# HyHuang1995/sp_orb_slam

Measured on AMD Instinct MI355X. Metric: frames/sec SuperPoint extract (752x480, 1k kpts), higher is better.
Workload: dtype f32

## Files before the change

### sp_orb_slam_amd/csrc/conv_f32.hip

```cpp
#include <type_traits>
#include <utility>

#include "spfe_kernels.h"
#include "../../include/spfe_exact_math.h"

namespace spfe {

typedef float f32x16 __attribute__((ext_vector_type(16)));

template <int KS, int TH>
struct Geo {
  static constexpr int HALO = KS / 2;
  static constexpr int ROWS = TH + 2 * HALO;
  static constexpr int COLS = 32 + 2 * HALO;
  static constexpr int ROWP = (KS == 3) ? 36 : 32;
  static constexpr int PLANE_RAW = ROWS * ROWP;
  static constexpr int PLANE = PLANE_RAW + ((2 - PLANE_RAW % 8) + 8) % 8;
};

typedef int i32x4 __attribute__((ext_vector_type(4)));
#define SPFE_OOB 0x80000000u

template <int NITER, int NWITER>
struct Pipe {
  float4 va[NITER];
  float4 vw[NWITER];
  int dst[NITER];
  unsigned voff[NITER];
  unsigned woff[NWITER];
  __amdgpu_buffer_rsrc_t rin, rw;
  const float *at[8];
  const float *bBase;
  float *nA, *nW;
};

template <int NR, int NT>
struct EpiCtx {
  __amdgpu_buffer_rsrc_t rout;
  unsigned rbase[NR][NT];
  float bias[NT];
  int xlim;
  unsigned pixstep;
};

__device__ __forceinline__ float max4_finite(float a, float b, float c, float d) {
  float m;
  asm("v_max3_f32 %0, %1, %2, %3\n\tv_max_f32 %0, %0, %4" : "=&v"(m) : "v"(a), "v"(b), "v"(c), "v"(d));
  return m;
}

template <int MT, int NT, bool POOL, bool RELU, int E>
__device__ __forceinline__ void epi_store(const EpiCtx<POOL ? MT / 2 : MT, NT> &e, const f32x16 (&acc)[MT][NT]) {
  constexpr int NEPI_ = POOL ? (MT / 2) * NT * 8 : MT * NT * 16;
  if constexpr (E >= NEPI_) {
    return;
  } else if constexpr (!POOL) {
    constexpr int j = E / (MT * 16), i = (E / 16) % MT, r = E % 16;
    constexpr int xr = (r & 3) + 8 * (r >> 2);
    float v = acc[i][j][r] + e.bias[j];
    if (RELU) v = v > 0.0f ? v : 0.0f;
    const unsigned off = xr < e.xlim ? e.rbase[i][j] : SPFE_OOB;
    __builtin_amdgcn_raw_buffer_store_b32(__float_as_int(v), e.rout, off, xr * e.pixstep, 0);
  } else {
    constexpr int ip = E / (NT * 8), j = (E / 8) % NT, r = 2 * (E % 8), i0 = 2 * ip;
    constexpr int xr = (r & 3) + 8 * (r >> 2);
    const float m = max4_finite(acc[i0][j][r], acc[i0][j][r + 1], acc[i0 + 1][j][r], acc[i0 + 1][j][r + 1]);
    float v = m + e.bias[j];
    if (RELU) v = v > 0.0f ? v : 0.0f;
    const unsigned off = xr < e.xlim ? e.rbase[ip][j] : SPFE_OOB;
    __builtin_amdgcn_raw_buffer_store_b32(__float_as_int(v), e.rout, off, (xr >> 1) * e.pixstep, 0);
  }
}

constexpr int F1_PROWS = 12, F1_PCOLS = 36, F1_PATCH = F1_PROWS * F1_PCOLS;

template <int NITER>
struct Fuse1a {
  float4 w[9], bias;
  float px[9];
  float4 o;
  unsigned pb[NITER];
  const float *patch;
  float *patch_next;
  const float *wsrc;
  const float *bsrc;
  __amdgpu_buffer_rsrc_t rimg;
  unsigned poff[2];
  unsigned pidx[2];
  unsigned pval[2];
  bool fill;
};
struct NoFuse {};

constexpr int F1_SUBS = 10;
template <int NITER, int IT, int SUB, int PLANE, int NWITER>
__device__ __forceinline__ void fuse_piece(Fuse1a<NITER> &z, Pipe<NITER, NWITER> &c) {
  if constexpr (SUB == 0) {
    const unsigned b = z.pb[IT] == ~0u ? 0u : z.pb[IT];
#pragma unroll
    for (int t = 0; t < 9; ++t) z.px[t] = z.patch[b + (t / 3) * F1_PCOLS + t % 3];
  } else if constexpr (SUB <= 8) {
    constexpr int j = (SUB - 1) / 2, half = (SUB - 1) % 2;
    float acc = half == 0 ? 0.0f : (j == 0 ? z.o.x : (j == 1 ? z.o.y : (j == 2 ? z.o.z : z.o.w)));
#pragma unroll
    for (int t = half * 5; t < (half == 0 ? 5 : 9); ++t) {
      const float wt = j == 0 ? z.w[t].x : (j == 1 ? z.w[t].y : (j == 2 ? z.w[t].z : z.w[t].w));
      acc = __builtin_fmaf(z.px[t], wt, acc);
    }
    if constexpr (half == 1) {
      const float bj = j == 0 ? z.bias.x : (j == 1 ? z.bias.y : (j == 2 ? z.bias.z : z.bias.w));
      acc = acc + bj;
      acc = acc > 0.0f ? acc : 0.0f;
      if (c.voff[IT] == SPFE_OOB) acc = 0.0f;
    }
    if constexpr (j == 0) z.o.x = acc;
    else if constexpr (j == 1) z.o.y = acc;
    else if constexpr (j == 2) z.o.z = acc;
    else z.o.w = acc;
  } else {
    float *d = c.nA + c.dst[IT];
    d[0] = z.o.x;
    d[PLANE] = z.o.y;
    d[2 * PLANE] = z.o.z;
    d[3 * PLANE] = z.o.w;
  }
}

template <int STEP, int NSTEP, bool FIRST, int KC, int KS, int MT, int NT, int PLANE, int ROWP, int NITER,
          int NWITER, bool POOL, bool RELU, bool FUSE, class FZ>
__device__ __forceinline__ void k_steps(float (&a)[2][MT], float (&bb)[2][NT], f32x16 (&acc)[MT][NT],
                                        const f32x16 (&accPrev)[MT][NT], Pipe<NITER, NWITER> &c,
                                        const EpiCtx<POOL ? MT / 2 : MT, NT> &e, FZ &fz) {
  if constexpr (STEP < NSTEP) {
    constexpr int NLDA = FUSE ? 0 : NITER;
    constexpr int NLD = NLDA + NWITER;
    constexpr int L0 = 1, W0 = NSTEP - NLD - 1;
    constexpr int NEPI = POOL ? (MT / 2) * NT * 8 : MT * NT * 16;
    constexpr int EPS = (NEPI + (NSTEP - 3)) / (NSTEP - 2);
    constexpr int cur = STEP & 1, nxt = cur ^ 1;
    static_assert(L0 + NLD <= W0, "loads and LDS writes of a stage must not overlap");
    constexpr int M = MT * NT;
    if constexpr (STEP >= 1) __builtin_amdgcn_s_waitcnt(0xC07F);
#pragma unroll
    for (int m = 0; m < M; ++m) {
      if (m == 0) {
        if constexpr (STEP + 1 < NSTEP) {
          constexpr int tap = (STEP + 1) / (KC / 2), t = (STEP + 1) % (KC / 2);
          constexpr int dy = tap / KS, dx = tap % KS;
#pragma unroll
          for (int i = 0; i < MT; ++i) {
            if constexpr (KC / 2 <= 8) a[nxt][i] = c.at[t][(i + dy) * ROWP + dx];
            else a[nxt][i] = c.at[0][(2 * t) * PLANE + (i + dy) * ROWP + dx];
          }
#pragma unroll
          for (int j = 0; j < NT; ++j) bb[nxt][j] = c.bBase[j * (KS * KS * KC * 32) + (tap * KC + 2 * t) * 32];
        }
      }
      if (m == 1 % M) {
        if constexpr (STEP >= L0 && STEP - L0 < NLD) {
          constexpr int it = STEP - L0;
          if constexpr (it < NLDA) {
            const i32x4 v = __builtin_amdgcn_raw_buffer_load_b128(c.rin, c.voff[it], 0, 0);
            c.va[it] = make_float4(__int_as_float(v.x), __int_as_float(v.y), __int_as_float(v.z), __int_as_float(v.w));
          } else {
            constexpr int wi = it - NLDA;
            const i32x4 v = __builtin_amdgcn_raw_buffer_load_b128(c.rw, c.woff[wi], 0, 0);
            c.vw[wi] = make_float4(__int_as_float(v.x), __int_as_float(v.y), __int_as_float(v.z), __int_as_float(v.w));
          }
        }
      }
      if (m == 2 % M) {
        if constexpr (FIRST && STEP >= 1) {
          constexpr int e0 = (STEP - 1) * EPS;
          [&]<int... Qs>(std::integer_sequence<int, Qs...>) {
            (epi_store<MT, NT, POOL, RELU, e0 + Qs>(e, accPrev), ...);
          }(std::make_integer_sequence<int, EPS>{});
        }
      }
      if (m == 3 % M) {
        if constexpr (STEP >= W0 && STEP - W0 < NLD) {
          constexpr int it = STEP - W0;
          if constexpr (it < NLDA) {
            float *d = c.nA + c.dst[it];
            d[0] = c.va[it].x;
            d[PLANE] = c.va[it].y;
            d[2 * PLANE] = c.va[it].z;
            d[3 * PLANE] = c.va[it].w;
          } else {
            constexpr int wi = it - NLDA;
            *reinterpret_cast<float4 *>(reinterpret_cast<char *>(c.nW) + c.woff[wi]) = c.vw[wi];
          }
        }
      }
      if (m == 1 % M) {
        if constexpr (FUSE) {
          constexpr int F0 = 12;
          static_assert(L0 + NLD <= F0 && F0 + F1_SUBS * NITER <= NSTEP, "fused conv1a schedule does not fit the stage");
          if constexpr (STEP >= F0 && STEP < F0 + F1_SUBS * NITER)
            fuse_piece<NITER, (STEP - F0) / F1_SUBS, (STEP - F0) % F1_SUBS, PLANE, NWITER>(fz, c);
        }
      }
      if (m == 3 % M) {
        if constexpr (FUSE) {
          static_assert(58 < W0, "fused conv1a schedule does not fit the stage");
          if constexpr (STEP >= 2 && STEP < 11) fz.w[STEP - 2] = *reinterpret_cast<const float4 *>(fz.wsrc + (STEP - 2) * 64);
          if constexpr (STEP == 11) fz.bias = *reinterpret_cast<const float4 *>(fz.bsrc);
          if constexpr (STEP == 50) {
            if (fz.fill) {
              fz.pval[0] = __builtin_amdgcn_raw_buffer_load_b8(fz.rimg, fz.poff[0], 0, 0);
              fz.pval[1] = __builtin_amdgcn_raw_buffer_load_b8(fz.rimg, fz.poff[1], 0, 0);
            }
          }
          if constexpr (STEP == 58) {
            if (fz.fill) {
              if (fz.pidx[0] < F1_PATCH) fz.patch_next[fz.pidx[0]] = spfe_pixel_to_float((uint8_t)fz.pval[0]);
              if (fz.pidx[1] < F1_PATCH) fz.patch_next[fz.pidx[1]] = spfe_pixel_to_float((uint8_t)fz.pval[1]);
            }
          }
        }
      }
      __builtin_amdgcn_sched_barrier(0);
      {
        const int i = m / NT, j = m % NT;
        if constexpr (FIRST && STEP == 0) {
          f32x16 z;
#pragma unroll
          for (int r = 0; r < 16; ++r) z[r] = 0.0f;
          acc[i][j] = __builtin_amdgcn_mfma_f32_32x32x2f32(a[cur][i], bb[cur][j], z, 0, 0, 0);
        } else {
          acc[i][j] = __builtin_amdgcn_mfma_f32_32x32x2f32(a[cur][i], bb[cur][j], acc[i][j], 0, 0, 0);
        }
      }
      __builtin_amdgcn_sched_barrier(0);
    }
    k_steps<STEP + 1, NSTEP, FIRST, KC, KS, MT, NT, PLANE, ROWP, NITER, NWITER, POOL, RELU, FUSE, FZ>(a, bb, acc, accPrev, c, e, fz);
  }
}

template <int LAYER, int CIN, int KS, int KC, int WM, int WN, int MT, int NT, bool POOL, bool RELU>
__global__ __launch_bounds__(64 * WM * WN, 1) void conv_f32_kernel(ConvParams p) {
  constexpr int TH = WM * MT;
  using G = Geo<KS, TH>;
  constexpr int TAPS = KS * KS;
  constexpr int NCHUNK = CIN / KC;
  constexpr int PLANE = G::PLANE;
  constexpr int ROWP = G::ROWP;
  constexpr int BUF = KC * PLANE + TAPS * KC * 64;
  static_assert(WM * WN == 4 || WM * WN == 8, "4 or 8 waves per workgroup");
  constexpr int NTHR = 64 * WM * WN;
  static_assert(WN * NT == 2, "64 output channels per workgroup");
  static_assert(!POOL || MT % 2 == 0, "pooling needs row pairs per wave");
  static_assert((KC * PLANE) % 4 == 0 && BUF % 4 == 0, "weight slabs must stay 16B aligned");
  constexpr int Q = KC / 4;
  constexpr int NITEM = G::ROWS * G::COLS * Q;
  constexpr int NITER = (NITEM + NTHR - 1) / NTHR;
  constexpr int NW4 = TAPS * KC * 16;
  constexpr int NWITER = (NW4 + NTHR - 1) / NTHR;
  constexpr int NSTEP = TAPS * (KC / 2);
  constexpr int SLAB_BYTES = TAPS * KC * 64 * 4;

  constexpr bool FUSE = LAYER == 2;
  static_assert(!FUSE || (CIN == 64 && KS == 3 && KC == 16 && TH == 8), "fused conv1a is conv1b's first operand");
  using FZ = typename std::conditional<FUSE, Fuse1a<NITER>, NoFuse>::type;

  extern __shared__ __attribute__((aligned(16))) float smem[];

  const int tid = threadIdx.x;
  const int lane = tid & 63;
  const int wave = __builtin_amdgcn_readfirstlane(tid >> 6);
  const int hi = lane >> 5, l31 = lane & 31;
  const int wm = wave % WM, wn = wave / WM;
  const int H = p.H, W = p.W;

  const int total = p.nblk * p.tiles_x * p.tiles_y * p.B;
  const int first = p.item_lo, count = (p.item_hi > 0 ? p.item_hi : total) - first;
  const int xcd = blockIdx.x & 7, gi = blockIdx.x >> 3, gper = gridDim.x >> 3;
  const int lo = first + (int)((long)count * xcd / 8), hi_w = first + (int)((long)count * (xcd + 1) / 8);
  int w = lo + gi;
  if (w >= hi_w) return;

  int i_nb, i_tx, i_ty, i_b;
  {
    int t = w;
    i_nb = t % p.nblk; t /= p.nblk;
    i_tx = t % p.tiles_x; t /= p.tiles_x;
    i_ty = t % p.tiles_y; i_b = t / p.tiles_y;
  }
  int d_nb, d_tx, d_ty, d_b;
  {
    int t = gper;
    d_nb = t % p.nblk; t /= p.nblk;
    d_tx = t % p.tiles_x; t /= p.tiles_x;
    d_ty = t % p.tiles_y; d_b = t / p.tiles_y;
  }

  const unsigned in_pix_bytes = (unsigned)p.in_stride * 4u;
  const unsigned frame_in_bytes = (unsigned)H * W * in_pix_bytes;
  const int Ho = POOL ? H >> 1 : H, Wo = POOL ? W >> 1 : W;
  const unsigned out_pix_bytes = (unsigned)p.out_stride * 4u;
  const unsigned frame_out_bytes = (unsigned)Ho * Wo * out_pix_bytes;

  Pipe<NITER, NWITER> c;
  int prow[NITER], pcol[NITER];
  unsigned pqb[NITER];
#pragma unroll
  for (int it = 0; it < NITER; ++it) {
    const int i = tid + it * NTHR;
    const int qq = i % Q, pix = i / Q;
    prow[it] = i < NITEM ? pix / G::COLS - G::HALO : (1 << 20);
    pcol[it] = pix % G::COLS - G::HALO;
    pqb[it] = qq * 16;
    c.dst[it] = i < NITEM ? (qq * 4) * PLANE + (pix / G::COLS) * ROWP + pix % G::COLS
                          : (ROWP > G::COLS ? (tid % G::ROWS) * ROWP + G::COLS : G::PLANE_RAW);
  }
#pragma unroll
  for (int it = 0; it < NWITER; ++it) c.woff[it] = ((tid + it * NTHR) % NW4) * 16;

  auto aim_tile = [&](int tx, int ty) {
#pragma unroll
    for (int it = 0; it < NITER; ++it) {
      const int gy = ty * TH + prow[it], gx = tx * 32 + pcol[it];
      c.voff[it] = ((unsigned)gy < (unsigned)H && (unsigned)gx < (unsigned)W)
                       ? (unsigned)(gy * W + gx) * in_pix_bytes + pqb[it]
                       : SPFE_OOB;
    }
  };
  auto aim_stage = [&](int nb, int b, int chunk, bool valid) {
    const float *base = p.in + (size_t)b * H * W * p.in_stride + p.in_choff + chunk * KC;
    c.rin = __builtin_amdgcn_make_buffer_rsrc(const_cast<float *>(base), 0, valid ? frame_in_bytes : 0u, 0x00020000);
    const float *wb = p.wpack + ((size_t)nb * NCHUNK + chunk) * (TAPS * KC * 64);
    c.rw = __builtin_amdgcn_make_buffer_rsrc(const_cast<float *>(wb), 0, valid ? (unsigned)SLAB_BYTES : 0u, 0x00020000);
  };

  aim_tile(i_tx, i_ty);
  aim_stage(i_nb, i_b, 0, true);
  FZ fz;
  [[maybe_unused]] float *sP = smem + 2 * BUF;
  [[maybe_unused]] int pcur = 0;
  [[maybe_unused]] int php[2] = {0, 0}, pwp[2] = {0, 0};
  if constexpr (FUSE) {
    const int qq = tid % Q;
#pragma unroll
    for (int it = 0; it < NITER; ++it) {
      const int i = tid + it * 256, pix = i / Q;
      fz.pb[it] = i < NITEM ? (unsigned)((pix / G::COLS) * F1_PCOLS + pix % G::COLS) : ~0u;
    }
#pragma unroll
    for (int k = 0; k < 2; ++k) {
      const int i = tid + k * 256;
      fz.pidx[k] = i < F1_PATCH ? (unsigned)i : 0xffffu;
      php[k] = i / F1_PCOLS;
      pwp[k] = i % F1_PCOLS;
      fz.poff[k] = SPFE_OOB;
      fz.pval[k] = 0u;
    }
    fz.fill = false;
    fz.patch = sP;
    fz.patch_next = sP + F1_PATCH;
    fz.rimg = __builtin_amdgcn_make_buffer_rsrc(const_cast<uint8_t *>(p.img), 0, 0u, 0x00020000);
    fz.wsrc = p.w1a + qq * 4;
    fz.bsrc = p.b1a + qq * 4;
    {
      const uint8_t *ib = p.img + (size_t)i_b * H * W;
#pragma unroll
      for (int k = 0; k < 2; ++k) {
        const int gy = i_ty * TH - 2 + php[k], gx = i_tx * 32 - 2 + pwp[k];
        const bool in = (unsigned)gy < (unsigned)H && (unsigned)gx < (unsigned)W;
        if (fz.pidx[k] < F1_PATCH) sP[fz.pidx[k]] = in ? spfe_pixel_to_float(ib[(size_t)gy * W + gx]) : 0.0f;
      }
    }
    __syncthreads();
#pragma unroll
    for (int t = 0; t < 9; ++t) fz.w[t] = *reinterpret_cast<const float4 *>(fz.wsrc + t * 64);
    fz.bias = *reinterpret_cast<const float4 *>(fz.bsrc);
    c.nA = smem;
    [&]<int... I>(std::integer_sequence<int, I...>) {
      (fuse_piece<NITER, I / F1_SUBS, I % F1_SUBS, PLANE, NWITER>(fz, c), ...);
    }(std::make_integer_sequence<int, F1_SUBS * NITER>{});
  } else {
#pragma unroll
    for (int it = 0; it < NITER; ++it) {
      const i32x4 v = __builtin_amdgcn_raw_buffer_load_b128(c.rin, c.voff[it], 0, 0);
      c.va[it] = make_float4(__int_as_float(v.x), __int_as_float(v.y), __int_as_float(v.z), __int_as_float(v.w));
    }
  }
#pragma unroll
  for (int it = 0; it < NWITER; ++it) {
    const i32x4 v = __builtin_amdgcn_raw_buffer_load_b128(c.rw, c.woff[it], 0, 0);
    c.vw[it] = make_float4(__int_as_float(v.x), __int_as_float(v.y), __int_as_float(v.z), __int_as_float(v.w));
  }
  if constexpr (!FUSE) {
#pragma unroll
    for (int it = 0; it < NITER; ++it) {
      float *d = smem + c.dst[it];
      d[0] = c.va[it].x;
      d[PLANE] = c.va[it].y;
      d[2 * PLANE] = c.va[it].z;
      d[3 * PLANE] = c.va[it].w;
    }
  }
#pragma unroll
  for (int it = 0; it < NWITER; ++it)
    *reinterpret_cast<float4 *>(reinterpret_cast<char *>(smem + KC * PLANE) + c.woff[it]) = c.vw[it];
  __syncthreads();

  f32x16 accA[MT][NT], accB[MT][NT];
#pragma unroll
  for (int i = 0; i < MT; ++i)
#pragma unroll
    for (int j = 0; j < NT; ++j)
#pragma unroll
      for (int r = 0; r < 16; ++r) { accA[i][j][r] = 0.0f; accB[i][j][r] = 0.0f; }

  constexpr int NR = POOL ? MT / 2 : MT;
  using Epi = EpiCtx<NR, NT>;
  Epi epi;
  epi.rout = __builtin_amdgcn_make_buffer_rsrc(p.out, 0, 0u, 0x00020000);
#pragma unroll
  for (int j = 0; j < NT; ++j) {
    epi.bias[j] = 0.0f;
#pragma unroll
    for (int q = 0; q < NR; ++q) epi.rbase[q][j] = SPFE_OOB;
  }
  epi.xlim = 0; epi.pixstep = out_pix_bytes;
  bool more = true;

  auto aim_epi = [&](Epi &e, int nb, int tx, int ty, int b) {
    float *obase = p.out + (size_t)b * Ho * Wo * p.out_stride + p.out_choff;
    e.rout = __builtin_amdgcn_make_buffer_rsrc(obase, 0, frame_out_bytes, 0x00020000);
    const int y0 = ty * TH + wm * MT, x0 = tx * 32 + 4 * hi;
    e.xlim = W - x0;
    e.pixstep = out_pix_bytes;
    const int ylim = H - y0;
    const unsigned rowstep = (unsigned)Wo * out_pix_bytes;
#pragma unroll
    for (int j = 0; j < NT; ++j) {
      const int co = nb * 64 + (wn * NT + j) * 32 + l31;
      const unsigned pix = POOL ? (unsigned)((y0 >> 1) * Wo + (x0 >> 1)) : (unsigned)(y0 * W + x0);
      const unsigned obase = pix * out_pix_bytes + (unsigned)co * 4u;
#pragma unroll
      for (int q = 0; q < NR; ++q)
        e.rbase[q][j] = (co < p.cout_real && (POOL ? 2 * q : q) < ylim) ? obase + q * rowstep : SPFE_OOB;
      e.bias[j] = p.bias[co];
    }
  };

  Epi epi_next;
  auto run_tile = [&](f32x16(&acc)[MT][NT], const f32x16(&accPrev)[MT][NT]) {
    int n_nb = i_nb + d_nb, n_tx = i_tx + d_tx, n_ty = i_ty + d_ty, n_b = i_b + d_b;
    if (n_nb >= p.nblk) { n_nb -= p.nblk; ++n_tx; }
    if (n_tx >= p.tiles_x) { n_tx -= p.tiles_x; ++n_ty; }
    if (n_ty >= p.tiles_y) { n_ty -= p.tiles_y; ++n_b; }
    const bool have_next_item = w + gper < hi_w;
    aim_epi(epi_next, i_nb, i_tx, i_ty, i_b);
    auto stage = [&]<bool FIRST>(std::bool_constant<FIRST>, const int chunk) {
      const bool last = chunk == NCHUNK - 1;
      if (!last) {
        aim_stage(i_nb, i_b, chunk + 1, true);
      } else {
        aim_tile(n_tx, n_ty);
        aim_stage(n_nb, n_b, 0, have_next_item);
      }
      if constexpr (FUSE) {
        const int produced = last ? 0 : chunk + 1;
        const int qq = tid % Q;
        fz.wsrc = p.w1a + produced * KC + qq * 4;
        fz.bsrc = p.b1a + produced * KC + qq * 4;
        fz.patch = sP + (last ? pcur ^ 1 : pcur) * F1_PATCH;
        fz.patch_next = sP + (pcur ^ 1) * F1_PATCH;
        fz.fill = chunk == NCHUNK - 2 && have_next_item;
        if (fz.fill) {
          fz.rimg = __builtin_amdgcn_make_buffer_rsrc(const_cast<uint8_t *>(p.img) + (size_t)n_b * H * W, 0,
                                                      (unsigned)(H * W), 0x00020000);
#pragma unroll
          for (int k = 0; k < 2; ++k) {
            const int gy = n_ty * TH - 2 + php[k], gx = n_tx * 32 - 2 + pwp[k];
            fz.poff[k] = ((unsigned)gy < (unsigned)H && (unsigned)gx < (unsigned)W) ? (unsigned)(gy * W + gx) : SPFE_OOB;
          }
        }
      }
      const int buf = chunk & 1;
      float *cA = smem + buf * BUF;
      c.nA = smem + (buf ^ 1) * BUF;
      c.nW = c.nA + KC * PLANE;
#pragma unroll
      for (int t = 0; t < (KC / 2 <= 8 ? KC / 2 : 1); ++t)
        c.at[t] = cA + (2 * t + hi) * PLANE + (wm * MT) * ROWP + l31;
      c.bBase = cA + KC * PLANE + (wn * NT) * (TAPS * KC * 32) + hi * 32 + l31;
      float a[2][MT], bb[2][NT];
#pragma unroll
      for (int i = 0; i < MT; ++i) a[0][i] = c.at[0][i * ROWP];
#pragma unroll
      for (int j = 0; j < NT; ++j) bb[0][j] = c.bBase[j * (TAPS * KC * 32)];
      k_steps<0, NSTEP, FIRST, KC, KS, MT, NT, PLANE, ROWP, NITER, NWITER, POOL, RELU, FUSE, FZ>(a, bb, acc, accPrev, c, epi, fz);
      __syncthreads();
    };
    static_assert(NCHUNK >= 2 && NCHUNK % 2 == 0, "the stage that carries the epilogue is not the tile's last; buf = chunk & 1");
    stage(std::true_type{}, 0);
#pragma unroll 1
    for (int chunk = 1; chunk < NCHUNK; ++chunk) stage(std::false_type{}, chunk);
    epi = epi_next;
    if constexpr (FUSE) pcur ^= 1;
    more = have_next_item;
    w += gper;
    i_nb = n_nb; i_tx = n_tx; i_ty = n_ty; i_b = n_b;
  };

  bool lastA = true;
  while (true) {
    run_tile(accA, accB);
    lastA = true;
    if (!more) break;
    run_tile(accB, accA);
    lastA = false;
    if (!more) break;
  }
  {
    constexpr int NEPI = POOL ? (MT / 2) * NT * 8 : MT * NT * 16;
    auto flush = [&](const f32x16(&acc)[MT][NT]) {
      [&]<int... E>(std::integer_sequence<int, E...>) {
        (epi_store<MT, NT, POOL, RELU, E>(epi, acc), ...);
      }(std::make_integer_sequence<int, NEPI>{});
    };
    if (lastA) flush(accA); else flush(accB);
  }
}

template <int LAYER, int CIN, int KS, int KC, int WM, int WN, int MT, int NT, bool POOL, bool RELU>
static hipError_t launch_one(const ConvParams &p, hipStream_t s) {
  constexpr int TH = WM * MT;
  using G = Geo<KS, TH>;
  constexpr size_t lds = (2 * (size_t)(KC * G::PLANE + KS * KS * KC * 64) + (LAYER == 2 ? 2 * F1_PATCH : 0)) * sizeof(float);
  static_assert(lds <= 160 * 1024, "double buffer must fit the 160 KB LDS");
  auto k = conv_f32_kernel<LAYER, CIN, KS, KC, WM, WN, MT, NT, POOL, RELU>;
  static bool attr_done[64] = {};
  int dev = 0;
  (void)hipGetDevice(&dev);
  if (dev < 0 || dev >= 64 || !attr_done[dev]) {
    hipError_t e = hipFuncSetAttribute(reinterpret_cast<const void *>(k),
                                       hipFuncAttributeMaxDynamicSharedMemorySize, (int)lds);
    if (e != hipSuccess) return e;
    if (dev >= 0 && dev < 64) attr_done[dev] = true;
  }
  const int total = p.nblk * p.tiles_x * p.tiles_y * p.B;
  int grid = p.num_cus > 0 ? p.num_cus : 256;
  grid &= ~7;
  if (grid < 8) grid = 8;
  (void)total;
  hipLaunchKernelGGL(k, dim3(grid), dim3(64 * WM * WN), lds, s, p);
  return hipGetLastError();
}

int conv_kc(int ksize) { return ksize == 3 ? 16 : 64; }
int conv_tile_rows(int tile_mode) { return tile_mode == 1 ? 4 : (tile_mode == 2 || tile_mode == 4 ? 16 : (tile_mode == 3 ? 2 : 8)); }

hipError_t launch_conv_f32(const ConvParams &p, int cin, int ksize, bool pool, bool relu,
                           int tile_mode, int layer_tag, hipStream_t s) {
  const bool small_tile = tile_mode == 1;
  if (tile_mode == 3 && ksize == 3 && relu && !pool) {
    if (cin == 64) return launch_one<0, 64, 3, 16, 2, 2, 1, 1, false, true>(p, s);
    if (cin == 128) return launch_one<0, 128, 3, 16, 2, 2, 1, 1, false, true>(p, s);
    return hipErrorInvalidValue;
  }
  if (tile_mode == 4 && ksize == 3 && relu && pool && cin == 64 && layer_tag == 1)
    return launch_one<1, 64, 3, 16, 4, 1, 4, 2, true, true>(p, s);
  if (tile_mode == 2 && ksize == 3 && relu) {
    if (layer_tag == 1 && cin == 64 && pool) return launch_one<1, 64, 3, 16, 8, 1, 2, 2, true, true>(p, s);
    if (cin == 64 && pool) return launch_one<0, 64, 3, 16, 8, 1, 2, 2, true, true>(p, s);
    if (cin == 64 && !pool) return launch_one<0, 64, 3, 16, 8, 1, 2, 2, false, true>(p, s);
    if (cin == 128 && pool) return launch_one<0, 128, 3, 16, 8, 1, 2, 2, true, true>(p, s);
    if (cin == 128 && !pool) return launch_one<0, 128, 3, 16, 8, 1, 2, 2, false, true>(p, s);
    return hipErrorInvalidValue;
  }
  if (layer_tag == 1 && cin == 64 && ksize == 3 && pool && relu && !small_tile)
    return launch_one<1, 64, 3, 16, 4, 1, 2, 2, true, true>(p, s);
  if (layer_tag == 2 && cin == 64 && ksize == 3 && pool && relu && !small_tile && p.img && p.w1a && p.b1a)
    return launch_one<2, 64, 3, 16, 4, 1, 2, 2, true, true>(p, s);
#define SPFE_CONV(CIN_, KS_, KC_, WM_, WN_, MT_, NT_, POOL_, RELU_)                       \
  if (cin == CIN_ && ksize == KS_ && pool == POOL_ && relu == RELU_ &&                    \
      small_tile == (WM_ * MT_ == 4))                                                     \
    return launch_one<0, CIN_, KS_, KC_, WM_, WN_, MT_, NT_, POOL_, RELU_>(p, s);
  SPFE_CONV(64, 3, 16, 4, 1, 2, 2, true, true)
  SPFE_CONV(64, 3, 16, 4, 1, 2, 2, false, true)
  SPFE_CONV(128, 3, 16, 4, 1, 2, 2, true, true)
  SPFE_CONV(128, 3, 16, 4, 1, 2, 2, false, true)
  SPFE_CONV(64, 3, 16, 2, 2, 2, 1, true, true)
  SPFE_CONV(64, 3, 16, 2, 2, 2, 1, false, true)
  SPFE_CONV(128, 3, 16, 2, 2, 2, 1, true, true)
  SPFE_CONV(128, 3, 16, 2, 2, 2, 1, false, true)
  SPFE_CONV(256, 1, 64, 2, 2, 2, 1, false, false)
#undef SPFE_CONV
  return hipErrorInvalidValue;
}

__global__ __launch_bounds__(256) void conv1a_kernel(const uint8_t *__restrict__ img,
                                                     const float *__restrict__ w9x64,
                                                     const float *__restrict__ b64,
                                                     float *__restrict__ out, int B, int H, int W,
                                                     int tiles_x, int tiles_y) {
  constexpr int TH = 8, TW = 32;
  __shared__ float sI[(TH + 2) * (TW + 2)];
  const int tid = threadIdx.x;
  int wg = blockIdx.x;
  const int tx = wg % tiles_x;
  wg /= tiles_x;
  const int ty = wg % tiles_y;
  const int b = wg / tiles_y;
  const int tx0 = tx * TW, ty0 = ty * TH;
  const uint8_t *ib = img + (size_t)b * H * W;
  for (int i = tid; i < (TH + 2) * (TW + 2); i += 256) {
    const int row = i / (TW + 2), col = i % (TW + 2);
    const int gy = ty0 + row - 1, gx = tx0 + col - 1;
    float v = 0.0f;
    if ((unsigned)gy < (unsigned)H && (unsigned)gx < (unsigned)W)
      v = (float)ib[(size_t)gy * W + gx] * (1.0f / 255.0f);
    sI[i] = v;
  }
  const int c4 = tid & 15;
  float4 w[9];
#pragma unroll
  for (int t = 0; t < 9; ++t) w[t] = *reinterpret_cast<const float4 *>(w9x64 + t * 64 + c4 * 4);
  const float4 bias = *reinterpret_cast<const float4 *>(b64 + c4 * 4);
  __syncthreads();
  const int psub = tid >> 4;
#pragma unroll 4
  for (int it = 0; it < 16; ++it) {
    const int pix = it * 16 + psub;
    const int row = pix >> 5, col = pix & 31;
    float4 a = make_float4(0.f, 0.f, 0.f, 0.f);
#pragma unroll
    for (int t = 0; t < 9; ++t) {
      const float x = sI[(row + t / 3) * (TW + 2) + col + t % 3];
      a.x = fmaf(x, w[t].x, a.x);
      a.y = fmaf(x, w[t].y, a.y);
      a.z = fmaf(x, w[t].z, a.z);
      a.w = fmaf(x, w[t].w, a.w);
    }
    a.x += bias.x;
    a.y += bias.y;
    a.z += bias.z;
    a.w += bias.w;
    a.x = a.x > 0.f ? a.x : 0.f;
    a.y = a.y > 0.f ? a.y : 0.f;
    a.z = a.z > 0.f ? a.z : 0.f;
    a.w = a.w > 0.f ? a.w : 0.f;
    const int gy = ty0 + row, gx = tx0 + col;
    if (gy < H && gx < W)
      *reinterpret_cast<float4 *>(out + (((size_t)b * H + gy) * W + gx) * 64 + c4 * 4) = a;
  }
}

__global__ __launch_bounds__(256) void pool2x2_f32_kernel(const float4 *__restrict__ in, float4 *__restrict__ out, int B, int Ho,
                                                          int Wo, int c4) {
  const size_t n = (size_t)B * Ho * Wo * c4;
  for (size_t i = (size_t)blockIdx.x * 256 + threadIdx.x; i < n; i += (size_t)gridDim.x * 256) {
    const int c = (int)(i % c4);
    size_t t = i / c4;
    const int x = (int)(t % Wo);
    t /= Wo;
    const int y = (int)(t % Ho), b = (int)(t / Ho);
    const size_t W = (size_t)Wo * 2, base = (((size_t)b * Ho * 2 + 2 * y) * W + 2 * x) * c4 + c;
    const float4 a = in[base], bq = in[base + c4], cq = in[base + W * c4], d = in[base + W * c4 + c4];
    float4 o;
    o.x = fmaxf(fmaxf(a.x, bq.x), fmaxf(cq.x, d.x));
    o.y = fmaxf(fmaxf(a.y, bq.y), fmaxf(cq.y, d.y));
    o.z = fmaxf(fmaxf(a.z, bq.z), fmaxf(cq.z, d.z));
    o.w = fmaxf(fmaxf(a.w, bq.w), fmaxf(cq.w, d.w));
    out[i] = o;
  }
}
hipError_t launch_pool2x2_f32(const float *in, float *out, int B, int H, int W, int C, hipStream_t s) {
  if ((H & 1) || (W & 1) || (C & 3)) return hipErrorInvalidValue;
  const size_t n = (size_t)B * (H / 2) * (W / 2) * (C / 4);
  const int grid = (int)((n + 255) / 256 < 4096 ? (n + 255) / 256 : 4096);
  hipLaunchKernelGGL(pool2x2_f32_kernel, dim3(grid), dim3(256), 0, s, reinterpret_cast<const float4 *>(in),
                     reinterpret_cast<float4 *>(out), B, H / 2, W / 2, C / 4);
  return hipGetLastError();
}

hipError_t launch_conv1a(const uint8_t *img, const float *w9x64, const float *b64, float *out, int B,
                         int H, int W, hipStream_t s) {
  const int tiles_x = (W + 31) / 32, tiles_y = (H + 7) / 8;
  hipLaunchKernelGGL(conv1a_kernel, dim3(tiles_x * tiles_y * B), dim3(256), 0, s, img, w9x64, b64,
                     out, B, H, W, tiles_x, tiles_y);
  return hipGetLastError();
}

}
```

Measured before the change: 2176.

## Hand over LDS buffers early inside the K-step loop of the conv kernel

Moves the stage-end barrier into the last K step and preloads the next stage's first operands from the other LDS buffer before that step, so consecutive stages chain without a full __syncthreads bubble and operand reload. Buffer pointers now flip by a signed delta, and the next tile's load offsets and buffer resources are computed in spare slots during the current stage instead of at stage start. Pointers are also retyped as LDS address-space pointers so the compiler emits ds instructions directly. This raises register pressure and adds a tight schedule whose ordering must stay correct.

```diff
diff --git a/sp_orb_slam_amd/csrc/conv_f32.hip b/sp_orb_slam_amd/csrc/conv_f32.hip
--- a/sp_orb_slam_amd/csrc/conv_f32.hip
+++ b/sp_orb_slam_amd/csrc/conv_f32.hip
@@ -19,19 +19,33 @@
 };
 
 typedef int i32x4 __attribute__((ext_vector_type(4)));
+#ifndef SPFE_CONV_HANDOVER
+#define SPFE_CONV_HANDOVER 1
+#endif
+template <int LAYER, int MT, int NT>
+inline constexpr bool kHandoverEarly = SPFE_CONV_HANDOVER == 2 || (SPFE_CONV_HANDOVER == 1 && MT * NT > 1);
+#ifndef SPFE_CONV_PROBE
+#define SPFE_CONV_PROBE(C, POINT)
+#define SPFE_CONV_PROBE_FIELDS
+#endif
 #define SPFE_OOB 0x80000000u
 
+typedef __attribute__((address_space(3))) float *lds_ptr;
+typedef const __attribute__((address_space(3))) float *lds_cptr;
 template <int NITER, int NWITER>
 struct Pipe {
   float4 va[NITER];
   float4 vw[NWITER];
   int dst[NITER];
   unsigned voff[NITER];
+  unsigned nvoff[NITER];
   unsigned woff[NWITER];
   __amdgpu_buffer_rsrc_t rin, rw;
-  const float *at[8];
-  const float *bBase;
-  float *nA, *nW;
+  lds_cptr at[8];
+  lds_cptr bBase;
+  lds_ptr nA, nW;
+  int dlt;
+  SPFE_CONV_PROBE_FIELDS
 };
 
 template <int NR, int NT>
@@ -118,7 +132,7 @@
     else if constexpr (j == 2) z.o.z = acc;
     else z.o.w = acc;
   } else {
-    float *d = c.nA + c.dst[IT];
+    lds_ptr d = c.nA + c.dst[IT];
     d[0] = z.o.x;
     d[PLANE] = z.o.y;
     d[2 * PLANE] = z.o.z;
@@ -127,10 +141,10 @@
 }
 
 template <int STEP, int NSTEP, bool FIRST, int KC, int KS, int MT, int NT, int PLANE, int ROWP, int NITER,
-          int NWITER, bool POOL, bool RELU, bool FUSE, class FZ>
+          int NWITER, bool POOL, bool RELU, bool FUSE, bool HO, class FZ, class AIM>
 __device__ __forceinline__ void k_steps(float (&a)[2][MT], float (&bb)[2][NT], f32x16 (&acc)[MT][NT],
                                         const f32x16 (&accPrev)[MT][NT], Pipe<NITER, NWITER> &c,
-                                        const EpiCtx<POOL ? MT / 2 : MT, NT> &e, FZ &fz) {
+                                        const EpiCtx<POOL ? MT / 2 : MT, NT> &e, FZ &fz, AIM &aim_next) {
   if constexpr (STEP < NSTEP) {
     constexpr int NLDA = FUSE ? 0 : NITER;
     constexpr int NLD = NLDA + NWITER;
@@ -139,8 +153,18 @@
     constexpr int EPS = (NEPI + (NSTEP - 3)) / (NSTEP - 2);
     constexpr int cur = STEP & 1, nxt = cur ^ 1;
     static_assert(L0 + NLD <= W0, "loads and LDS writes of a stage must not overlap");
+    static_assert(W0 + NLD - 1 == NSTEP - 2, "the stage's last LDS write stands one step in front of its last K step");
+    constexpr int NAT = KC / 2 <= 8 ? KC / 2 : 1;
+    static_assert(NSTEP % NAT == 0 && NAT + 1 < NSTEP && L0 + NLD <= NSTEP - 3, "early hand-over: pointer slots");
     constexpr int M = MT * NT;
+    if constexpr (STEP == 0) { SPFE_CONV_PROBE(c, 3); }
     if constexpr (STEP >= 1) __builtin_amdgcn_s_waitcnt(0xC07F);
+    if constexpr (STEP == NSTEP / 2) { SPFE_CONV_PROBE(c, 4); }
+    if constexpr (HO && STEP == NSTEP - 1) {
+      __builtin_amdgcn_s_barrier();
+      SPFE_CONV_PROBE(c, 1);
+      __builtin_amdgcn_sched_barrier(0);
+    }
 #pragma unroll
     for (int m = 0; m < M; ++m) {
       if (m == 0) {
@@ -154,6 +178,12 @@
           }
 #pragma unroll
           for (int j = 0; j < NT; ++j) bb[nxt][j] = c.bBase[j * (KS * KS * KC * 32) + (tap * KC + 2 * t) * 32];
+        } else if constexpr (HO) {
+          static_assert(NSTEP % 2 == 0, "the operand sets alternate");
+#pragma unroll
+          for (int i = 0; i < MT; ++i) a[nxt][i] = c.at[0][i * ROWP];
+#pragma unroll
+          for (int j = 0; j < NT; ++j) bb[nxt][j] = c.bBase[j * (KS * KS * KC * 32)];
         }
       }
       if (m == 1 % M) {
@@ -176,25 +206,42 @@
             (epi_store<MT, NT, POOL, RELU, e0 + Qs>(e, accPrev), ...);
           }(std::make_integer_sequence<int, EPS>{});
         }
+        if constexpr (HO) {
+          if constexpr (NAT > 1 && STEP >= NSTEP - NAT) c.at[STEP - (NSTEP - NAT)] += c.dlt;
+          if constexpr (NAT == 1 && STEP == NSTEP - 2) c.at[0] += c.dlt;
+          if constexpr (STEP == NSTEP - 2) c.bBase += c.dlt;
+        }
       }
       if (m == 3 % M) {
         if constexpr (STEP >= W0 && STEP - W0 < NLD) {
           constexpr int it = STEP - W0;
           if constexpr (it < NLDA) {
-            float *d = c.nA + c.dst[it];
+            lds_ptr d = c.nA + c.dst[it];
             d[0] = c.va[it].x;
             d[PLANE] = c.va[it].y;
             d[2 * PLANE] = c.va[it].z;
             d[3 * PLANE] = c.va[it].w;
           } else {
             constexpr int wi = it - NLDA;
-            *reinterpret_cast<float4 *>(reinterpret_cast<char *>(c.nW) + c.woff[wi]) = c.vw[wi];
+            typedef float f32x4 __attribute__((ext_vector_type(4)));
+            *(__attribute__((address_space(3))) f32x4 *)((__attribute__((address_space(3))) char *)c.nW + c.woff[wi]) =
+                f32x4{c.vw[wi].x, c.vw[wi].y, c.vw[wi].z, c.vw[wi].w};
           }
+        }
+      }
+      if (m == 1 % M) {
+        if constexpr (HO) {
+          static_assert(L0 + NLD + NITER <= NSTEP - 3 - NITER, "early hand-over: offset slots");
+          if constexpr (FIRST && STEP >= L0 + NLD && STEP < L0 + NLD + NITER) aim_next.template operator()<1, STEP - L0 - NLD>();
+          if constexpr (!FUSE && STEP >= NSTEP - 3 - NITER && STEP < NSTEP - 3) aim_next.template operator()<2, STEP - (NSTEP - 3 - NITER)>();
+          if constexpr (FUSE && STEP == NSTEP - 2)
+            [&]<int... I>(std::integer_sequence<int, I...>) { (aim_next.template operator()<2, I>(), ...); }(std::make_integer_sequence<int, NITER>{});
+          if constexpr (STEP == NSTEP - 3) aim_next.template operator()<0, 0>();
         }
       }
       if (m == 1 % M) {
         if constexpr (FUSE) {
-          constexpr int F0 = 12;
+          constexpr int F0 = HO ? 10 : 12;
           static_assert(L0 + NLD <= F0 && F0 + F1_SUBS * NITER <= NSTEP, "fused conv1a schedule does not fit the stage");
           if constexpr (STEP >= F0 && STEP < F0 + F1_SUBS * NITER)
             fuse_piece<NITER, (STEP - F0) / F1_SUBS, (STEP - F0) % F1_SUBS, PLANE, NWITER>(fz, c);
@@ -219,6 +266,13 @@
           }
         }
       }
+      if (m == 3 % M) {
+        if constexpr (HO && STEP == NSTEP - 1) {
+          c.nA -= c.dlt;
+          c.nW -= c.dlt;
+          c.dlt = -c.dlt;
+        }
+      }
       __builtin_amdgcn_sched_barrier(0);
       {
         const int i = m / NT, j = m % NT;
@@ -231,9 +285,15 @@
           acc[i][j] = __builtin_amdgcn_mfma_f32_32x32x2f32(a[cur][i], bb[cur][j], acc[i][j], 0, 0, 0);
         }
       }
+      if (m == 0) {
+        if constexpr (STEP == 0) { SPFE_CONV_PROBE(c, 0); }
+      }
+      if (m == M - 1) {
+        if constexpr (STEP == NSTEP - 1) { SPFE_CONV_PROBE(c, 2); }
+      }
       __builtin_amdgcn_sched_barrier(0);
     }
-    k_steps<STEP + 1, NSTEP, FIRST, KC, KS, MT, NT, PLANE, ROWP, NITER, NWITER, POOL, RELU, FUSE, FZ>(a, bb, acc, accPrev, c, e, fz);
+    k_steps<STEP + 1, NSTEP, FIRST, KC, KS, MT, NT, PLANE, ROWP, NITER, NWITER, POOL, RELU, FUSE, HO, FZ, AIM>(a, bb, acc, accPrev, c, e, fz, aim_next);
   }
 }
 
@@ -260,6 +320,7 @@
   constexpr int SLAB_BYTES = TAPS * KC * 64 * 4;
 
   constexpr bool FUSE = LAYER == 2;
+  constexpr bool HO = kHandoverEarly<LAYER, MT, NT>;
   static_assert(!FUSE || (CIN == 64 && KS == 3 && KC == 16 && TH == 8), "fused conv1a is conv1b's first operand");
   using FZ = typename std::conditional<FUSE, Fuse1a<NITER>, NoFuse>::type;
 
@@ -316,16 +377,20 @@
 #pragma unroll
   for (int it = 0; it < NWITER; ++it) c.woff[it] = ((tid + it * NTHR) % NW4) * 16;
 
+  unsigned pbase[NITER];
+#pragma unroll
+  for (int it = 0; it < NITER; ++it) pbase[it] = (unsigned)(prow[it] * W + pcol[it]) * in_pix_bytes + pqb[it];
+  auto piece_off = [&](int it, int tx, int ty) __attribute__((always_inline)) {
+    const unsigned off = pbase[it] + (unsigned)(ty * TH * W + tx * 32) * in_pix_bytes;
+    const int gy = ty * TH + prow[it], gx = tx * 32 + pcol[it];
+    if constexpr (FUSE) return ((unsigned)gy < (unsigned)H && (unsigned)gx < (unsigned)W) ? off : SPFE_OOB;
+    else return (unsigned)gx < (unsigned)W ? off : SPFE_OOB;
+  };
   auto aim_tile = [&](int tx, int ty) {
 #pragma unroll
-    for (int it = 0; it < NITER; ++it) {
-      const int gy = ty * TH + prow[it], gx = tx * 32 + pcol[it];
-      c.voff[it] = ((unsigned)gy < (unsigned)H && (unsigned)gx < (unsigned)W)
-                       ? (unsigned)(gy * W + gx) * in_pix_bytes + pqb[it]
-                       : SPFE_OOB;
-    }
+    for (int it = 0; it < NITER; ++it) c.voff[it] = piece_off(it, tx, ty);
   };
-  auto aim_stage = [&](int nb, int b, int chunk, bool valid) {
+  auto aim_stage = [&](int nb, int b, int chunk, bool valid) __attribute__((always_inline)) {
     const float *base = p.in + (size_t)b * H * W * p.in_stride + p.in_choff + chunk * KC;
     c.rin = __builtin_amdgcn_make_buffer_rsrc(const_cast<float *>(base), 0, valid ? frame_in_bytes : 0u, 0x00020000);
     const float *wb = p.wpack + ((size_t)nb * NCHUNK + chunk) * (TAPS * KC * 64);
@@ -373,7 +438,7 @@
 #pragma unroll
     for (int t = 0; t < 9; ++t) fz.w[t] = *reinterpret_cast<const float4 *>(fz.wsrc + t * 64);
     fz.bias = *reinterpret_cast<const float4 *>(fz.bsrc);
-    c.nA = smem;
+    c.nA = (lds_ptr)smem;
     [&]<int... I>(std::integer_sequence<int, I...>) {
       (fuse_piece<NITER, I / F1_SUBS, I % F1_SUBS, PLANE, NWITER>(fz, c), ...);
     }(std::make_integer_sequence<int, F1_SUBS * NITER>{});
@@ -403,6 +468,21 @@
   for (int it = 0; it < NWITER; ++it)
     *reinterpret_cast<float4 *>(reinterpret_cast<char *>(smem + KC * PLANE) + c.woff[it]) = c.vw[it];
   __syncthreads();
+  float opa[2][MT], opb[2][NT];
+  if constexpr (HO) {
+    aim_stage(i_nb, i_b, 1, true);
+#pragma unroll
+    for (int t = 0; t < (KC / 2 <= 8 ? KC / 2 : 1); ++t)
+      c.at[t] = (lds_cptr)(smem + (2 * t + hi) * PLANE + (wm * MT) * ROWP + l31);
+    c.bBase = (lds_cptr)(smem + KC * PLANE + (wn * NT) * (TAPS * KC * 32) + hi * 32 + l31);
+    c.dlt = BUF;
+    c.nA = (lds_ptr)(smem + BUF);
+    c.nW = c.nA + KC * PLANE;
+#pragma unroll
+    for (int i = 0; i < MT; ++i) opa[0][i] = c.at[0][i * ROWP];
+#pragma unroll
+    for (int j = 0; j < NT; ++j) opb[0][j] = c.bBase[j * (TAPS * KC * 32)];
+  }
 
   f32x16 accA[MT][NT], accB[MT][NT];
 #pragma unroll
@@ -446,21 +526,35 @@
   };
 
   Epi epi_next;
-  auto run_tile = [&](f32x16(&acc)[MT][NT], const f32x16(&accPrev)[MT][NT]) {
+  auto run_tile = [&](f32x16(&acc)[MT][NT], const f32x16(&accPrev)[MT][NT]) __attribute__((always_inline)) {
     int n_nb = i_nb + d_nb, n_tx = i_tx + d_tx, n_ty = i_ty + d_ty, n_b = i_b + d_b;
     if (n_nb >= p.nblk) { n_nb -= p.nblk; ++n_tx; }
     if (n_tx >= p.tiles_x) { n_tx -= p.tiles_x; ++n_ty; }
     if (n_ty >= p.tiles_y) { n_ty -= p.tiles_y; ++n_b; }
     const bool have_next_item = w + gper < hi_w;
     aim_epi(epi_next, i_nb, i_tx, i_ty, i_b);
-    auto stage = [&]<bool FIRST>(std::bool_constant<FIRST>, const int chunk) {
+    auto stage = [&]<bool FIRST>(std::bool_constant<FIRST>, const int chunk) __attribute__((always_inline)) {
       const bool last = chunk == NCHUNK - 1;
-      if (!last) {
-        aim_stage(i_nb, i_b, chunk + 1, true);
+      if constexpr (!HO) {
+        if (!last) {
+          aim_stage(i_nb, i_b, chunk + 1, true);
+        } else {
+          aim_tile(n_tx, n_ty);
+          aim_stage(n_nb, n_b, 0, have_next_item);
+        }
       } else {
-        aim_tile(n_tx, n_ty);
-        aim_stage(n_nb, n_b, 0, have_next_item);
-      }
+      }
+      auto aim_next = [&]<int KIND, int IT>() __attribute__((always_inline)) {
+        if constexpr (KIND == 0) {
+          const int c2 = chunk + 2;
+          const bool wrap = c2 >= NCHUNK;
+          aim_stage(wrap ? n_nb : i_nb, wrap ? n_b : i_b, wrap ? c2 - NCHUNK : c2, wrap ? have_next_item : true);
+        } else if constexpr (KIND == 1) {
+          c.nvoff[IT] = piece_off(IT, n_tx, n_ty);
+        } else {
+          c.voff[IT] = chunk == NCHUNK - 2 ? c.nvoff[IT] : c.voff[IT];
+        }
+      };
       if constexpr (FUSE) {
         const int produced = last ? 0 : chunk + 1;
         const int qq = tid % Q;
@@ -479,21 +573,25 @@
           }
         }
       }
-      const int buf = chunk & 1;
-      float *cA = smem + buf * BUF;
-      c.nA = smem + (buf ^ 1) * BUF;
-      c.nW = c.nA + KC * PLANE;
-#pragma unroll
-      for (int t = 0; t < (KC / 2 <= 8 ? KC / 2 : 1); ++t)
-        c.at[t] = cA + (2 * t + hi) * PLANE + (wm * MT) * ROWP + l31;
-      c.bBase = cA + KC * PLANE + (wn * NT) * (TAPS * KC * 32) + hi * 32 + l31;
-      float a[2][MT], bb[2][NT];
-#pragma unroll
-      for (int i = 0; i < MT; ++i) a[0][i] = c.at[0][i * ROWP];
-#pragma unroll
-      for (int j = 0; j < NT; ++j) bb[0][j] = c.bBase[j * (TAPS * KC * 32)];
-      k_steps<0, NSTEP, FIRST, KC, KS, MT, NT, PLANE, ROWP, NITER, NWITER, POOL, RELU, FUSE, FZ>(a, bb, acc, accPrev, c, epi, fz);
-      __syncthreads();
+      if constexpr (!HO) {
+        const int buf = chunk & 1;
+        float *cA = smem + buf * BUF;
+        c.nA = (lds_ptr)(smem + (buf ^ 1) * BUF);
+        c.nW = c.nA + KC * PLANE;
+#pragma unroll
+        for (int t = 0; t < (KC / 2 <= 8 ? KC / 2 : 1); ++t)
+          c.at[t] = (lds_cptr)(cA + (2 * t + hi) * PLANE + (wm * MT) * ROWP + l31);
+        c.bBase = (lds_cptr)(cA + KC * PLANE + (wn * NT) * (TAPS * KC * 32) + hi * 32 + l31);
+#pragma unroll
+        for (int i = 0; i < MT; ++i) opa[0][i] = c.at[0][i * ROWP];
+#pragma unroll
+        for (int j = 0; j < NT; ++j) opb[0][j] = c.bBase[j * (TAPS * KC * 32)];
+      }
+      k_steps<0, NSTEP, FIRST, KC, KS, MT, NT, PLANE, ROWP, NITER, NWITER, POOL, RELU, FUSE, HO, FZ>(opa, opb, acc, accPrev, c, epi, fz, aim_next);
+      if constexpr (!HO) {
+        __syncthreads();
+        SPFE_CONV_PROBE(c, 1);
+      }
     };
     static_assert(NCHUNK >= 2 && NCHUNK % 2 == 0, "the stage that carries the epilogue is not the tile's last; buf = chunk & 1");
     stage(std::true_type{}, 0);
```

Result: no change. 2187, median of 6 (+0.5%).
